# Kaixhin/Rainbow

Measured on AMD Instinct MI355X. Metric: gradient-steps/sec (batch=32, atoms=51), higher is better.
Workload: dtype f32; 1 GPU; pong-canonical-b32; architecture=canonical, batch_per_gpu=32, global_batch=32, atoms=51, actions=6, multi_step=3, replay_capacity_per_gpu=1000000, parallelism=single device

## Files before the change

### rainbow_amd/csrc/adam_body.h

```cpp
#pragma once
#include "rb_common.h"

struct ClipAdamArgs {
  float* p; float* g; float* m; float* v;
  int64_t n;
  const float* part; int nparts;
  float max_norm; float* norm_out;
  float w1, b2, w2, neg_step_size, bc2_sqrt, eps;
  const long long* step_dev;
  double lr, beta1, beta2;
  int64_t skip_lo4, skip_len4;
  const int32_t* batch_status;
  int64_t pair_mu4, pair_len4;
  unsigned hole_lo4, hole4;
  int pair_blk0;
  int pair_f4, pair_split_row;
  const float* pair_eout;
  const float* pair_ein;
  int32_t* pair_clipped;
};
__device__ __forceinline__ void rb_adam_elem(float& p, float& g, float& m, float& v, float coef, const ClipAdamArgs& a) {
  g = g * coef;
  m = fmaf(a.w1, g - m, m);
  v = v * a.b2 + a.w2 * g * g;
  const float denom = sqrtf(v) / a.bc2_sqrt + a.eps;
  p = p + a.neg_step_size * (m / denom);
}
__device__ __forceinline__ void rb_adam_quad(float4& P, float4& G, float4& M, float4& V, float coef, const ClipAdamArgs& a) {
  rb_adam_elem(P.x, G.x, M.x, V.x, coef, a);
  rb_adam_elem(P.y, G.y, M.y, V.y, coef, a);
  rb_adam_elem(P.z, G.z, M.z, V.z, coef, a);
  rb_adam_elem(P.w, G.w, M.w, V.w, coef, a);
}

struct rb_adam_req {
  float status;
  unsigned st_lo, st_hi;
  float pv[16];
};
__device__ __forceinline__ void rb_adam_hosted_request(const ClipAdamArgs& a, rb_adam_req& q) {
  const unsigned T = blockDim.x;
  q.status = 0.0f;
  if (a.batch_status) q.status = rb_ld1_buf(rb_make_buf(a.batch_status), 0, 0);
  const rb_buf bs = rb_make_buf(a.step_dev);
  q.st_lo = __builtin_bit_cast(unsigned, rb_ld1_buf(bs, 0, 0)); q.st_hi = __builtin_bit_cast(unsigned, rb_ld1_buf(bs, 4, 0));
  const rb_buf bpart = rb_make_buf(a.part);
#pragma unroll
  for (int u = 0; u < 16; ++u) {
    const int i = (int)threadIdx.x + u * (int)T;
    q.pv[u] = rb_ld1_buf(bpart, 4u * (unsigned)(i < a.nparts ? i : a.nparts - 1), 0);
  }
}
__device__ __forceinline__ bool rb_adam_hosted_prologue(ClipAdamArgs& a, int eb, const rb_adam_req& q, float* s_red16, float* coef_out) {
  const unsigned T = blockDim.x;
  float acc = 0.0f;
#pragma unroll
  for (int u = 0; u < 16; ++u)
    if ((int)threadIdx.x + u * (int)T < a.nparts) acc += q.pv[u];
  {
    const rb_buf bpart = rb_make_buf(a.part);
    for (int i0 = (int)threadIdx.x + 16 * (int)T; i0 < a.nparts; i0 += 16 * (int)T) {
      float pv[16];
#pragma unroll
      for (int u = 0; u < 16; ++u) {
        const int i = i0 + u * (int)T;
        pv[u] = rb_ld1_buf(bpart, 4u * (unsigned)(i < a.nparts ? i : a.nparts - 1), 0);
      }
#pragma unroll
      for (int u = 0; u < 16; ++u)
        if (i0 + u * (int)T < a.nparts) acc += pv[u];
    }
  }
  if (threadIdx.x == 0) {
    const double t = (double)(long long)(((unsigned long long)q.st_hi << 32) | q.st_lo);
    const double bc1 = 1.0 - pow(a.beta1, t), bc2 = 1.0 - pow(a.beta2, t);
    s_red16[16] = (float)(-(a.lr / bc1));
    s_red16[17] = (float)sqrt(bc2);
  }
  acc = rb_block_sum(acc, s_red16);
  if (rb_wave_uniform(__builtin_bit_cast(int, q.status)) != 0) {
    if (eb == 0 && threadIdx.x == 0 && a.norm_out) rb_st1_wt(a.norm_out, 0, 0.0f);
    return false;
  }
  const float total = sqrtf(acc);
  float coef = a.max_norm / (total + 1e-6f);
  if (coef > 1.0f) coef = 1.0f;
  if (eb == 0 && threadIdx.x == 0 && a.norm_out) rb_st1_wt(a.norm_out, 0, total);
  a.neg_step_size = s_red16[16];
  a.bc2_sqrt = s_red16[17];
  *coef_out = coef;
  return true;
}

__device__ __forceinline__ void rb_adam_hosted_pairs(ClipAdamArgs& a, int eb, int pb, float* s_red16) {
  constexpr int PU = 2;
  const unsigned T = blockDim.x;
  const unsigned len4 = (unsigned)a.pair_len4, mu4 = (unsigned)a.pair_mu4;
  const unsigned base = (unsigned)pb * (T * PU) + threadIdx.x;
  rb_adam_req q;
  rb_adam_hosted_request(a, q);
  const rb_buf beo = rb_make_buf(a.pair_eout), bei = rb_make_buf(a.pair_ein);
  float4 E[PU];
  float eo[PU];
#pragma unroll
  for (int u = 0; u < PU; ++u) {
    unsigned j = base + u * T;
    if (j >= len4) j = len4 - 1;
    const unsigned row = j / (unsigned)a.pair_f4, cq = j - row * (unsigned)a.pair_f4;
    eo[u] = rb_ld1_buf(beo, 4 * row, 0);
    E[u] = rb_ld4_buf(bei, 16 * (cq + ((int)row >= a.pair_split_row ? (unsigned)a.pair_f4 : 0u)), 0);
  }
  const rb_buf bp = rb_make_buf(a.p), bg = rb_make_buf(a.g), bm = rb_make_buf(a.m), bv = rb_make_buf(a.v);
  float4 P[PU], G[PU], M[PU], V[PU], P2[PU], M2[PU], V2[PU];
#pragma unroll
  for (int u = 0; u < PU; ++u) {
    unsigned j = base + u * T;
    if (j >= len4) j = len4 - 1;
    const unsigned i = mu4 + j, i2 = i + len4;
    P[u] = rb_ld4_buf(bp, 16 * i, 0); G[u] = rb_ld4_buf(bg, 16 * i, 0);
    M[u] = rb_ld4_buf(bm, 16 * i, 0); V[u] = rb_ld4_buf(bv, 16 * i, 0);
    P2[u] = rb_ld4_buf(bp, 16 * i2, 0); M2[u] = rb_ld4_buf(bm, 16 * i2, 0); V2[u] = rb_ld4_buf(bv, 16 * i2, 0);
  }
  float coef;
  if (!rb_adam_hosted_prologue(a, eb, q, s_red16, &coef)) return;
  if (pb == 0 && threadIdx.x == 0 && a.pair_clipped) rb_st1_wt(reinterpret_cast<float*>(a.pair_clipped), 0, __builtin_bit_cast(float, coef < 1.0f ? 1 : 0));
#pragma unroll
  for (int u = 0; u < PU; ++u) {
    const unsigned j = base + u * T;
    if (j >= len4) continue;
    const unsigned i = mu4 + j, i2 = i + len4;
    float4 pr;
    pr.x = eo[u] * E[u].x; pr.y = eo[u] * E[u].y; pr.z = eo[u] * E[u].z; pr.w = eo[u] * E[u].w;
    float4 G2;
    G2.x = G[u].x * pr.x; G2.y = G[u].y * pr.y; G2.z = G[u].z * pr.z; G2.w = G[u].w * pr.w;
    rb_adam_quad(P[u], G[u], M[u], V[u], coef, a);
    rb_adam_quad(P2[u], G2, M2[u], V2[u], coef, a);
    rb_st4_wt(a.p, 16 * i, P[u]); rb_st4_wt(a.m, 16 * i, M[u]); rb_st4_wt(a.v, 16 * i, V[u]);
    rb_st4_wt(a.p, 16 * i2, P2[u]); rb_st4_wt(a.m, 16 * i2, M2[u]); rb_st4_wt(a.v, 16 * i2, V2[u]);
    if (coef < 1.0f) { rb_st4_wt(a.g, 16 * i, G[u]); rb_st4_wt(a.g, 16 * i2, G2); }
  }
}

template <int UNROLL>
__device__ __forceinline__ void rb_adam_hosted_block(const ClipAdamArgs* ad, int eb, int nblk, float* s_red16 ) {
  ClipAdamArgs a = rb_ld_uniform(ad);
  const int nplain = a.hole4 > 0 ? a.pair_blk0 : nblk;
  if (eb >= nplain) {
    rb_adam_hosted_pairs(a, eb, eb - nplain, s_red16);
    return;
  }
  const unsigned T = blockDim.x;
  const unsigned n4 = (unsigned)(a.n >> 2);
  const unsigned hole_lo = a.hole4 > 0 ? a.hole_lo4 : n4, hole = a.hole4;
  const unsigned nv4 = n4 - hole;
  auto real_of = [&](unsigned j) { return j < hole_lo ? j : j + hole; };
  const unsigned base = (unsigned)eb * (T * UNROLL) + threadIdx.x;
  const rb_buf bp = rb_make_buf(a.p), bg = rb_make_buf(a.g), bm = rb_make_buf(a.m), bv = rb_make_buf(a.v);
  rb_adam_req q;
  rb_adam_hosted_request(a, q);
  float4 P[UNROLL], G[UNROLL], M[UNROLL], V[UNROLL];
#pragma unroll
  for (int u = 0; u < UNROLL; ++u) {
    unsigned j = base + u * T;
    if (j >= nv4) j = nv4 > 0 ? nv4 - 1 : 0;
    const unsigned i = real_of(j);
    P[u] = rb_ld4_buf(bp, 16 * i, 0); G[u] = rb_ld4_buf(bg, 16 * i, 0);
    M[u] = rb_ld4_buf(bm, 16 * i, 0); V[u] = rb_ld4_buf(bv, 16 * i, 0);
  }
  float coef;
  if (!rb_adam_hosted_prologue(a, eb, q, s_red16, &coef)) return;
#pragma unroll
  for (int u = 0; u < UNROLL; ++u) {
    const unsigned j = base + u * T;
    if (j >= nv4) continue;
    const unsigned i = real_of(j);
    rb_adam_quad(P[u], G[u], M[u], V[u], coef, a);
    rb_st4_wt(a.p, 16 * i, P[u]); rb_st4_wt(a.m, 16 * i, M[u]); rb_st4_wt(a.v, 16 * i, V[u]);
    if (coef < 1.0f) rb_st4_wt(a.g, 16 * i, G[u]);
  }
  if (eb == nplain - 1) {
    const int64_t t = ((a.n >> 2) << 2) + threadIdx.x;
    if (t < a.n) {
      const unsigned o = (unsigned)(4 * t);
      float p = rb_ld1_buf(bp, o, 0), g = rb_ld1_buf(bg, o, 0), m = rb_ld1_buf(bm, o, 0), v = rb_ld1_buf(bv, o, 0);
      rb_adam_elem(p, g, m, v, coef, a);
      rb_st1_wt(a.p, o, p); rb_st1_wt(a.m, o, m); rb_st1_wt(a.v, o, v);
      if (coef < 1.0f) rb_st1_wt(a.g, o, g);
    }
  }
}

int rb_launch_adam_pending(const ClipAdamArgs* args_dev, int blocks, void* stream);
```

### rainbow_amd/csrc/learner_internal.h

```cpp
#pragma once
#include "conv_fwd.h"
#include "conv_dx.h"
#include "conv_dw.h"
#include "noise_body.h"
#include "adam_body.h"
#include "learner_problems.h"
#include "noisy_linear.h"
#include "fc_gemm.h"
#include "act_path.h"
#include "rb_common.h"

#include <stdlib.h>

#include <math.h>
#include <string.h>

#include <new>

#define RB_HEAD_MAX_NZ 1408
typedef ConvGeom<8, 4, 84, 20> GeomC1;
typedef ConvGeom<4, 2, 20, 9> GeomC2;
typedef ConvGeom<3, 1, 9, 7> GeomC3;
typedef ConvGeom<5, 5, 84, 16> GeomD1;
typedef ConvGeom<5, 5, 16, 3> GeomD2;
// ... 2 lines not shown

struct ConvLayer {
  int cin, cout, ks, s, ih, oh;
  int K() const { return cin * ks * ks; }
  int P() const { return oh * oh; }
  int IP() const { return ih * ih; }
};

struct Layout {
  int B, Z, A, H, F, NZ, hist, nconv;
  ConvLayer conv[3];
  int64_t conv_w[3], conv_b[3];
  int64_t h_mu, h_sigma, h_bmu, h_bsigma, z_mu, z_sigma, z_bmu, z_bsigma;
  int64_t n_params;
  int64_t h_ein, h_eout, z_ein, z_eout, n_noise;
};

static int64_t align64(int64_t x) { return (x + 63) / 64 * 64; }

static int make_layout(const rb_learner_config_t* c, Layout* L) {
  RB_REQUIRE(c != nullptr, "learner config is NULL");
  RB_REQUIRE(c->batch >= 1 && c->batch <= 1024, "batch must be in [1,1024]");
  RB_REQUIRE(c->atoms >= 2 && c->atoms <= 256, "atoms must be in [2,256]");
  RB_REQUIRE(c->actions >= 1 && c->actions <= 64, "actions must be in [1,64]");
  RB_REQUIRE(c->atoms * (c->actions + 1) <= RB_HEAD_MAX_NZ, "atoms*(actions+1) must be <= %d (head kernel LDS rows)", RB_HEAD_MAX_NZ);
  RB_REQUIRE(c->history >= 1 && c->history <= 16, "history must be in [1,16]");
  RB_REQUIRE(c->hidden >= 1 && c->hidden <= 8192, "hidden must be in [1,8192]");
  RB_REQUIRE(c->architecture == 0 || c->architecture == 1, "architecture must be 0 (canonical) or 1 (data-efficient)");
  RB_REQUIRE(c->multi_step >= 1, "multi_step must be >= 1");
  RB_REQUIRE(c->v_max > c->v_min, "v_max must exceed v_min");
  memset(L, 0, sizeof(*L));
  L->B = c->batch; L->Z = c->atoms; L->A = c->actions; L->H = c->hidden; L->hist = c->history;
  L->NZ = L->Z + L->A * L->Z;
  if (c->architecture == 0) {
    L->nconv = 3;
    L->conv[0] = ConvLayer{c->history, 32, 8, 4, 84, 20};
    L->conv[1] = ConvLayer{32, 64, 4, 2, 20, 9};
    L->conv[2] = ConvLayer{64, 64, 3, 1, 9, 7};
    L->F = 3136;
  } else {
    L->nconv = 2;
    L->conv[0] = ConvLayer{c->history, 32, 5, 5, 84, 16};
    L->conv[1] = ConvLayer{32, 64, 5, 5, 16, 3};
    L->F = 576;
  }
  int64_t off = 0;
  for (int l = 0; l < L->nconv; ++l) {
    L->conv_w[l] = off; off = align64(off + (int64_t)L->conv[l].cout * L->conv[l].K());
    L->conv_b[l] = off; off = align64(off + L->conv[l].cout);
  }
  const int64_t H2 = 2 * L->H;
  L->h_mu = off; off = align64(off + H2 * L->F);
  L->h_sigma = off; off = align64(off + H2 * L->F);
  L->h_bmu = off; off = align64(off + H2);
  L->h_bsigma = off; off = align64(off + H2);
  L->z_mu = off; off = align64(off + (int64_t)L->NZ * L->H);
  L->z_sigma = off; off = align64(off + (int64_t)L->NZ * L->H);
  L->z_bmu = off; off = align64(off + L->NZ);
  L->z_bsigma = off; off = align64(off + L->NZ);
  L->n_params = off;
  int64_t n = 0;
  L->h_ein = n; n = align64(n + 2 * (int64_t)L->F);
  L->h_eout = n; n = align64(n + H2);
  L->z_ein = n; n = align64(n + H2);
  L->z_eout = n; n = align64(n + L->NZ);
  L->n_noise = n;
  return RB_OK;
}


static NetPtrs net_ptrs(const Layout& L, const float* params, const float* noise) {
  NetPtrs p;
  for (int l = 0; l < 3; ++l) {
    p.conv_w[l] = l < L.nconv ? params + L.conv_w[l] : nullptr;
    p.conv_b[l] = l < L.nconv ? params + L.conv_b[l] : nullptr;
  }
  p.h_mu = params + L.h_mu; p.h_sigma = params + L.h_sigma; p.h_bmu = params + L.h_bmu; p.h_bsigma = params + L.h_bsigma;
  p.z_mu = params + L.z_mu; p.z_sigma = params + L.z_sigma; p.z_bmu = params + L.z_bmu; p.z_bsigma = params + L.z_bsigma;
  p.h_ein = noise + L.h_ein; p.h_eout = noise + L.h_eout; p.z_ein = noise + L.z_ein; p.z_eout = noise + L.z_eout;
  return p;
}

struct RbOpts {
  int generic, fc_gemm, implicit_small, xs, act_fused, spec_draw, spec_stall, img_fast, conv_multi, conv_full, t16, dx_ipb, dw_ipb0, dw_ipb1, dw_ipb2;
};
static const struct { const char* key; int RbOpts::*field; int dflt; const char* what; } rb_opt_table[] = {
  {"generic", &RbOpts::generic, 0, "1: every contraction on the gemm_core.h fallback; 2: the noisy-linear layers only"},
  {"fc_gemm", &RbOpts::fc_gemm, -1, "hidden layer on the LDS-tiled GEMMs of fc_gemm.h: -1 = by shape (from 128 rows per net on), 1 = always, 0 = never"},
  {"implicit_small", &RbOpts::implicit_small, 0, "test hook: RB_LEARNER_IMPLICIT_SIGMA on hidden layers of any size"},
  {"xs", &RbOpts::xs, 0, "row splits of the hidden layer's input gradient: 0 = derived from the hidden size (ceil(2H / 256), at most 4)"},
  {"act_fused", &RbOpts::act_fused, 1, "Agent.act as ONE launch (0: the per-layer launches)"},
  {"spec_draw", &RbOpts::spec_draw, 0, "the early draw (opt-in: only append-free loops ever arm it)"},
  {"spec_stall", &RbOpts::spec_stall, 0, "test hook: the early draw's go flag is never stored, the gate in front of the pair expires"},
  {"img_fast", &RbOpts::img_fast, 1, "image-fastest block order of the conv launches (0: the order that image counts off a multiple of 8 get)"},
  {"conv_multi", &RbOpts::conv_multi, -1, "images per workgroup of the conv forward: -1 = by shape (from 256 images on), 0 = one"},
  {"conv_full", &RbOpts::conv_full, 1, "the first layer's whole-image kernel at large batches (0: the chunked kernel)"},
  {"t16", &RbOpts::t16, 1, "the canonical first layer's u8 forward on whole-K 16x16x4 tiles (0: the split-K kernel that history < 4 gets)"},
  {"dx_ipb", &RbOpts::dx_ipb, 0, "images per workgroup of the conv input gradients: 0 = by shape (from batch 64 on)"},
  {"dw_ipb0", &RbOpts::dw_ipb0, 0, "images per workgroup of conv layer 0 in the weight-gradient launch: 0 = by shape"},
  {"dw_ipb1", &RbOpts::dw_ipb1, 0, "... of conv layer 1"},
  {"dw_ipb2", &RbOpts::dw_ipb2, 0, "... of conv layer 2"},
};
static int rb_opts_parse(const char* s, RbOpts* o) {
  for (const auto& row : rb_opt_table) o->*row.field = row.dflt;
  while (s && *s) {
    const char* e = strchr(s, ',');
    const size_t n = e ? (size_t)(e - s) : strlen(s);
    const char* eq = (const char*)memchr(s, '=', n);
    RB_REQUIRE(eq != nullptr && eq > s, "RB_OPTS: entry '%.*s' is not key=value", (int)n, s);
    const size_t kl = (size_t)(eq - s);
    int RbOpts::*field = nullptr;
    for (const auto& row : rb_opt_table)
      if (strlen(row.key) == kl && strncmp(row.key, s, kl) == 0) field = row.field;
    RB_REQUIRE(field != nullptr, "RB_OPTS: unknown key '%.*s'", (int)kl, s);
    char* end = nullptr;
    const long v = strtol(eq + 1, &end, 10);
    RB_REQUIRE(end == s + n && end > eq + 1, "RB_OPTS: key '%.*s' needs an integer value", (int)kl, s);
    o->*field = (int)v;
    s = e ? e + 1 : s + n;
  }
  return RB_OK;
}

struct LearnerCaps {
  int fast_fc;
  int fast_conv;
  int hs, xs, ws[3];
  int wT[3];
  int gemm_ws;
};

struct rb_learner {
  rb_learner_config_t cfg;
  Layout L;
  float *p_online, *p_target, *grads, *n_online, *n_target;
  uint64_t seed;
  uint64_t noise_epoch;
  float* act[3];
  float* dact[3];
  float* hpart;
  float* h;
  float *feat_b, *h_b;
  float *feat_s, *h_s;
  int rows_s_cap;
  float* logits;
  float* dlogits;
  float* dlogitsT;
  float* dh;
  float* dhT;
  float* dfeat_part;
  int lazy_dfeat;
  int lazy_splits;
  RbOpts opt;
  float* gemm_part;
  unsigned* gemm_ctr;
  float* dw_part[3];
  float* conv_wT[3];
  float* log_ps_a;
  float* pns_a;
  float* m;
  int32_t* a_star;
  float* support;
  float* zero_noise;
  float* norm_part;
  int norm_conv_base;
  int norm_slots;
  unsigned long long* noise_ctr;
  NoiseJob* job_dev;
  unsigned* act_ctr;
  unsigned act_epoch;
  int n_cu;
  int rows_cap;
  LearnerCaps caps;
  int dw_slices[3];
  ImgSrc cur_src;
  int sink_done;
  const int32_t* batch_status;
  rb_replay_t* sink;
  const int64_t* sink_idx;
  int world;
  float* fact_local;
  const float* fact_all;
  int64_t fact_off[6];
  int64_t fact_stride;
// ... 36 lines not shown
```

### rainbow_amd/csrc/optimizer_host.h

```cpp
#pragma once
#include "learner_plan.h"

static int materialize_sigma(rb_learner* l, hipStream_t stream) {
  if (!l->sigma_implicit) return RB_OK;
  const Layout& L = l->L;
  const NetPtrs sn = net_ptrs(L, l->p_online, l->noise_snap);
  const int64_t len4 = (int64_t)2 * L.H * L.F / 4;
  RB_LAUNCH(k_materialize_sigma, dim3((unsigned)rb_div_up(len4, 256 * 4)), dim3(256), stream, l->grads, L.h_mu / 4, len4, L.F / 4, L.H,
            sn.h_eout, sn.h_ein, (const int32_t*)(l->status_copy + 2));
  RB_LAUNCH_CHECK();
  l->sigma_implicit = 0;
  return RB_OK;
}

static int flush_update(rb_learner* l, hipStream_t stream) {
  if (!l->adam_pending) return RB_OK;
  FusedDwAdamArgs f;
  memset(&f, 0, sizeof(f));
  ClipAdamArgs a = l->adam_args_host;
  int blocks = l->adam_blocks;
  if (a.pair_len4 > 0) {
    const int rc = rb_launch_adam_pending(l->adam_args_dev, blocks, stream);
    if (rc != RB_OK) return rc;
    l->adam_pending = 0;
    return RB_OK;
  }
  RB_LAUNCH_T("clip_adam:k_clip_adam", (k_clip_adam<4, true, false>), dim3((unsigned)blocks), dim3(256), stream, a, f);
  RB_LAUNCH_CHECK();
  l->adam_pending = 0;
  return RB_OK;
}

static int sumsq_pass(rb_learner* l, hipStream_t stream, int* nparts) {
  const int64_t n = l->L.n_params;
  *nparts = plan_sumsq_blocks(n);
  RB_LAUNCH(k_sumsq, dim3((unsigned)*nparts), dim3(256), stream, (const float*)l->grads, n, l->norm_part);
  RB_LAUNCH_CHECK();
  return RB_OK;
}

static bool attach_pending_pass(rb_learner* l, const rb_noise_job_t* job_in, int32_t batch, rb_noise_job_t* job_out) {
  memcpy(job_out, job_in, sizeof(*job_out));
  if (!l->adam_pending || batch > 256) return false;
  NoiseJob* nj = reinterpret_cast<NoiseJob*>(job_out);
  nj->adam_dev = l->adam_args_dev; nj->adam_blocks = l->adam_blocks;
  return true;
}

static int clip_adam_impl(rb_learner* l, float max_norm, float* exp_avg, float* exp_avg_sq, double lr, double beta1, double beta2,
                          double eps, int64_t step, float* norm_dev, hipStream_t stream, bool defer) {
  RB_REQUIRE(exp_avg != nullptr && exp_avg_sq != nullptr, "rb_learner_clip_adam: NULL moment buffer");
  RB_REQUIRE(step >= 1 || (step == 0 && l->step_ctr), "rb_learner_clip_adam: step is 1-based (0 = take it from the device counter set "
             "with rb_learner_set_step_counter)");
  const int64_t n = l->L.n_params;
  int nparts = l->norm_slots;
  if (!(max_norm < INFINITY) && norm_dev == nullptr) {
    nparts = 0;
  } else if (nparts <= 0) {
    const int rcs = sumsq_pass(l, stream, &nparts);
    if (rcs != RB_OK) return rcs;
  }
  l->norm_slots = 0;
  ClipAdamArgs a;
  memset(&a, 0, sizeof(a));
  a.p = l->p_online; a.g = l->grads; a.m = exp_avg; a.v = exp_avg_sq; a.n = n;
  a.part = l->norm_part; a.nparts = nparts; a.max_norm = max_norm; a.norm_out = norm_dev;
  const double bc1 = 1.0 - pow(beta1, (double)step), bc2 = 1.0 - pow(beta2, (double)step);
  a.w1 = (float)(1.0 - beta1); a.b2 = (float)beta2; a.w2 = (float)(1.0 - beta2);
  a.neg_step_size = (float)(-(lr / bc1)); a.bc2_sqrt = (float)sqrt(bc2); a.eps = (float)eps;
  a.step_dev = step == 0 ? l->step_ctr : nullptr; a.lr = lr; a.beta1 = beta1; a.beta2 = beta2;
  a.batch_status = l->status_copy;
  const int64_t n4 = n >> 2;
  RB_REQUIRE(n * 4 < (int64_t)0x7fffffff, "rb_learner_clip_adam: the flat parameter buffer must be smaller than 2 GiB");
  FusedDwAdamArgs f;
  memset(&f, 0, sizeof(f));
  a.skip_lo4 = 0; a.skip_len4 = 0;
  if (l->dw_deferred) {
    const Layout& L = l->L;
    const NetPtrs on = net_ptrs(L, l->p_online, l->n_online);
    FcDwPlan hp = fc_dw_plan(l, on, 1, l->dh, l->act[L.nconv - 1], L.B, 0);
    f.dw = hp.a;
    f.mu_off = L.h_mu; f.sigma_off = L.h_sigma;
    f.dw_x = hp.dw_x; f.n_tile_blocks = 2 * hp.dw_x * hp.dw_y;
    f.write_grads = (l->flags & RB_LEARNER_WRITE_FUSED_GRADS) ? 1 : 0;
    a.skip_lo4 = L.h_mu >> 2; a.skip_len4 = (L.h_bmu - L.h_mu) >> 2;
    const unsigned grid = (unsigned)(f.n_tile_blocks + rb_div_up(n4 - a.skip_len4 > 0 ? n4 - a.skip_len4 : 1, 256 * 4));
    RB_LAUNCH_T("clip_adam:k_clip_adam", (k_clip_adam<4, true, true>), dim3(grid), dim3(256), stream, a, f);
    l->dw_deferred = 0;
  } else {
    unsigned grid = (unsigned)rb_div_up(n4 > 0 ? n4 : 1, 256 * 4);
    const bool will_defer = defer && a.step_dev != nullptr && a.nparts > 0 && l->adam_args_dev != nullptr;
    if (l->sigma_implicit && will_defer) {
      const Layout& L = l->L;
      const NetPtrs sn = net_ptrs(L, l->p_online, l->noise_snap);
      a.pair_mu4 = L.h_mu / 4; a.pair_len4 = (int64_t)2 * L.H * L.F / 4;
      a.pair_f4 = L.F / 4; a.pair_split_row = L.H; a.pair_eout = sn.h_eout; a.pair_ein = sn.h_ein;
      a.pair_clipped = l->status_copy + 2;
      a.hole_lo4 = (unsigned)a.pair_mu4; a.hole4 = (unsigned)(2 * a.pair_len4);
      a.pair_blk0 = (int)rb_div_up(n4 - 2 * a.pair_len4 > 0 ? n4 - 2 * a.pair_len4 : 1, 256 * 4);
      grid = (unsigned)(a.pair_blk0 + rb_div_up(a.pair_len4, 256 * 2));
    } else if (l->sigma_implicit) {
      const int rcm = materialize_sigma(l, stream);
      if (rcm != RB_OK) return rcm;
    }
    if (will_defer) {
      if (!l->adam_args_valid || memcmp(&a, &l->adam_args_host, sizeof(a)) != 0) {
        RB_LAUNCH(k_store_adam_args, dim3(1), dim3(64), stream, a, l->adam_args_dev);
        RB_LAUNCH_CHECK();
        memcpy(&l->adam_args_host, &a, sizeof(a));
        l->adam_args_valid = 1;
      }
      l->adam_pending = 1;
      l->adam_blocks = (int)grid;
      return RB_OK;
    }
    RB_LAUNCH_T("clip_adam:k_clip_adam", (k_clip_adam<4, true, false>), dim3(grid), dim3(256), stream, a, f);
  }
  RB_LAUNCH_CHECK();
  return RB_OK;
}

extern "C" {

int rb_learner_flush(rb_learner_t* l, rb_stream_t stream) {
  RB_REQUIRE(l != nullptr, "rb_learner_flush: NULL handle");
  const int rc = flush_update(l, (hipStream_t)stream);
  if (rc != RB_OK) return rc;
  return materialize_sigma(l, (hipStream_t)stream);
}

int rb_learner_attach_pending(rb_learner_t* l, const rb_noise_job_t* job_in, int32_t batch, rb_noise_job_t* job_out) {
  if (!l || !job_in || !job_out) { rb_set_error("rb_learner_attach_pending: NULL argument"); return RB_ERR_INVALID; }
  return attach_pending_pass(l, job_in, batch, job_out) ? 1 : 0;
}
int rb_learner_pending_launched(rb_learner_t* l) {
  RB_REQUIRE(l != nullptr, "rb_learner_pending_launched: NULL handle");
  l->adam_pending = 0;
  return RB_OK;
}
int rb_debug_adam_pass(int32_t form, float* p, float* g, float* m, float* v, int64_t n, const float* part, int32_t nparts,
                       float max_norm, float* norm_out, const long long* step_dev, int64_t step, double lr, double beta1,
                       double beta2, double eps, const int32_t* batch_status, int64_t pair_mu4, int64_t pair_len4, int32_t pair_f4,
                       int32_t pair_split_row, const float* pair_eout, const float* pair_ein, int32_t* pair_clipped, void* args_dev,
                       rb_stream_t stream_) {
  hipStream_t stream = (hipStream_t)stream_;
  RB_REQUIRE(p && g && m && v && part && n >= 0 && n * 4 < (int64_t)0x7fffffff && nparts > 0, "rb_debug_adam_pass: bad buffers");
  RB_REQUIRE(form == 0 ? (step >= 1 && pair_len4 == 0) : (form == 1 && step_dev && args_dev), "rb_debug_adam_pass: bad form");
  static_assert(sizeof(ClipAdamArgs) <= 256, "rb_debug_adam_pass: args_dev is documented as 256 bytes");
  ClipAdamArgs a;
  memset(&a, 0, sizeof(a));
  a.p = p; a.g = g; a.m = m; a.v = v; a.n = n;
  a.part = part; a.nparts = nparts; a.max_norm = max_norm; a.norm_out = norm_out;
  const double bc1 = 1.0 - pow(beta1, (double)step), bc2 = 1.0 - pow(beta2, (double)step);
  a.w1 = (float)(1.0 - beta1); a.b2 = (float)beta2; a.w2 = (float)(1.0 - beta2);
  a.neg_step_size = (float)(-(lr / bc1)); a.bc2_sqrt = (float)sqrt(bc2); a.eps = (float)eps;
  a.step_dev = form == 1 ? step_dev : nullptr; a.lr = lr; a.beta1 = beta1; a.beta2 = beta2;
  a.batch_status = batch_status;
  const int64_t n4 = n >> 2;
  unsigned grid = (unsigned)rb_div_up(n4 > 0 ? n4 : 1, 256 * 4);
  if (form == 0) {
    FusedDwAdamArgs f;
    memset(&f, 0, sizeof(f));
    RB_LAUNCH((k_clip_adam<4, true, false>), dim3(grid), dim3(256), stream, a, f);
    RB_LAUNCH_CHECK();
    return RB_OK;
  }
  if (pair_len4 > 0) {
    RB_REQUIRE(pair_mu4 >= 0 && pair_mu4 + 2 * pair_len4 <= n4 && pair_f4 > 0 && pair_len4 % pair_f4 == 0 && pair_eout && pair_ein,
               "rb_debug_adam_pass: bad pair range");
    a.pair_mu4 = pair_mu4; a.pair_len4 = pair_len4; a.pair_f4 = pair_f4; a.pair_split_row = pair_split_row;
    a.pair_eout = pair_eout; a.pair_ein = pair_ein; a.pair_clipped = pair_clipped;
    a.hole_lo4 = (unsigned)pair_mu4; a.hole4 = (unsigned)(2 * pair_len4);
    a.pair_blk0 = (int)rb_div_up(n4 - 2 * pair_len4 > 0 ? n4 - 2 * pair_len4 : 1, 256 * 4);
    grid = (unsigned)(a.pair_blk0 + rb_div_up(pair_len4, 256 * 2));
  }
  RB_LAUNCH(k_store_adam_args, dim3(1), dim3(64), stream, a, reinterpret_cast<ClipAdamArgs*>(args_dev));
  RB_LAUNCH_CHECK();
  return rb_launch_adam_pending(reinterpret_cast<const ClipAdamArgs*>(args_dev), (int)grid, stream);
}

int rb_learner_clip_adam_deferred(rb_learner_t* l, float max_norm, float* exp_avg, float* exp_avg_sq, double lr, double beta1,
                                  double beta2, double eps, int64_t step, float* norm_dev, rb_stream_t stream) {
  RB_REQUIRE(l != nullptr, "rb_learner_clip_adam_deferred: NULL handle");
  const int rc = flush_update(l, (hipStream_t)stream);
  if (rc != RB_OK) return rc;
  return clip_adam_impl(l, max_norm, exp_avg, exp_avg_sq, lr, beta1, beta2, eps, step, norm_dev, (hipStream_t)stream,
                        (l->flags & RB_LEARNER_DEFER_UPDATE) != 0);
}

int rb_learner_clip_grad(rb_learner_t* l, float max_norm, float* norm_dev, rb_stream_t stream) {
  RB_REQUIRE(l != nullptr, "rb_learner_clip_grad: NULL handle");
  RB_FLUSH_UPDATE(l, stream);
  RB_MATERIALIZE_SIGMA(l, stream);
  if (l->dw_deferred) {
    rb_set_error("rb_learner_clip_grad: the last learn call left the hidden layer's weight gradient to the fused optimiser "
                 "pass (RB_LEARNER_FUSE_FC_H_DW); call rb_learner_clip_adam, or clear the flag before learning");
    return RB_ERR_STATE;
  }
  const int64_t n = l->L.n_params;
  int nblocks = plan_sumsq_blocks(n);
  int nparts = l->norm_slots;
  if (nparts > 0) {
    if (nblocks > 256) nblocks = 256;
  } else {
    const int rcs = sumsq_pass(l, (hipStream_t)stream, &nparts);
    if (rcs != RB_OK) return rcs;
  }
  l->norm_slots = 0;
  RB_LAUNCH(k_clip_scale, dim3((unsigned)nblocks), dim3(256), stream, l->grads, n, (const float*)l->norm_part, nparts,
            max_norm, norm_dev);
  RB_LAUNCH_CHECK();
  return RB_OK;
}

int rb_learner_clip_adam(rb_learner_t* l, float max_norm, float* exp_avg, float* exp_avg_sq, double lr, double beta1,
                         double beta2, double eps, int64_t step, float* norm_dev, rb_stream_t stream) {
  RB_REQUIRE(l != nullptr, "rb_learner_clip_adam: NULL handle");
  const int rc = flush_update(l, (hipStream_t)stream);
  if (rc != RB_OK) return rc;
  return clip_adam_impl(l, max_norm, exp_avg, exp_avg_sq, lr, beta1, beta2, eps, step, norm_dev, (hipStream_t)stream, false);
}

}
```

### rainbow_amd/csrc/replay.hip

```cpp
#include "noise_body.h"
#include "adam_body.h"
#include "replay_internal.h"
#include "replay_search.h"
#include "replay_append.h"
#include "replay_spec.h"
#include "replay_sample.h"
#include "replay_view.h"

#include <stdlib.h>
#include <string.h>

#include <new>

struct rb_replay {
  int64_t capacity;
  int32_t history, n;
  int32_t levels;
  int32_t streams;
  int64_t tree_start;
  int64_t tree_len;
  double omega;
  uint64_t seed;
  float scaling[64];
  float* tree;
// ... 352 lines not shown
int rb_replay_append_streams_dev(rb_replay_t* r, const float* states_dev, int32_t* timesteps_dev, const int32_t* actions_dev,
                                 const float* rewards_dev, const uint8_t* nonterminals_dev, rb_stream_t stream) {
  AppendRoundDev a;
  a.timestep = timesteps_dev; a.action = actions_dev; a.reward = rewards_dev; a.nonterminal = nonterminals_dev;
  const bool have = timesteps_dev && actions_dev && rewards_dev && nonterminals_dev;
  return append_round(r, "rb_replay_append_streams_dev", "append:k_append_streams_dev", states_dev, have ? &a : nullptr, stream);
}

int rb_replay_set_beta_source(rb_replay_t* r, const float* neg_beta_dev) {
  RB_REQUIRE(r != nullptr, "rb_replay_set_beta_source: NULL handle");
  r->neg_beta_dev = neg_beta_dev;
  return RB_OK;
}

int rb_replay_find(rb_replay_t* r, const double* values_dev, int32_t n, float* probs_dev, int64_t* data_idx_dev,
                   int64_t* tree_idx_dev, rb_stream_t stream) {
  RB_REQUIRE(r && values_dev && probs_dev && data_idx_dev && tree_idx_dev, "rb_replay_find: NULL argument");
  RB_SPEC_JOIN(r);
  if (n <= 0) return RB_OK;
  RB_LAUNCH(k_find, dim3((unsigned)rb_div_up(n, 256)), dim3(256), stream, view_of(r), values_dev, n, probs_dev,
            data_idx_dev, tree_idx_dev);
  RB_LAUNCH_CHECK();
  return RB_OK;
}

static int launch_gather(const ReplayView& v, int32_t batch, const int32_t* win, uint8_t* states_dev, uint8_t* next_states_dev,
                         rb_stream_t stream) {
  if (!states_dev || !next_states_dev) return RB_OK;
  RB_LAUNCH(k_gather_stacks, dim3((unsigned)(batch * 2 * v.history)), dim3(256), stream, v, batch, win, states_dev, next_states_dev);
  RB_LAUNCH_CHECK();
  return RB_OK;
}

static int sample_impl(rb_replay_t* r, int32_t batch, double priority_weight, const double* unit_uniforms_dev,
                       int32_t max_attempts, int64_t* tree_idx_dev, uint8_t* states_dev, uint8_t* next_states_dev,
                       int64_t* actions_dev, float* returns_dev, float* nonterminals_dev, float* weights_dev,
                       const rb_noise_job_t* noise_job, rb_stream_t stream) {
  RB_REQUIRE(r && tree_idx_dev && actions_dev && returns_dev && nonterminals_dev && weights_dev,
             "rb_replay_sample: NULL argument");
  RB_REQUIRE(batch >= 1 && batch <= r->max_batch, "rb_replay_sample: batch must be in [1,%d]", r->max_batch);
  RB_REQUIRE(max_attempts >= 1, "rb_replay_sample: max_attempts must be >= 1");
  RB_REQUIRE(r->capacity > (int64_t)r->history + r->n,
             "rb_replay_sample: capacity must exceed history + multi_step (no window can clear the write head otherwise: "
             "the reference's rejection loop, memory.py:128-132, would never end)");
  const int accept_armed = r->spec_accept_armed;
  r->spec_accept_armed = 0;
  int spec_mode = 0;
  int win_set = 0;
  if (r->spec_inflight) {
    const bool same = accept_armed && !rb_stream_capturing(stream) && unit_uniforms_dev == nullptr && r->spec_args.batch == batch && r->spec_args.beta == priority_weight &&
                      r->spec_args.max_attempts == max_attempts && r->spec_args.tree_idx == tree_idx_dev &&
                      r->spec_args.actions == actions_dev && r->spec_args.returns == returns_dev &&
                      r->spec_args.nonterm == nonterminals_dev && r->spec_args.weights == weights_dev;
    spec_mode = same ? 2 : 3;
    if (same) win_set = r->spec_args.win_set;
    r->spec_inflight = 0;
  }
  r->win_sel = win_set;
  ++r->mutations;
  int32_t* const win_cur = win_of(r, win_set);
  const ReplayView v = view_of(r);
  const float neg_beta = (float)(-priority_weight);
  NoiseJob job;
  memset(&job, 0, sizeof(job));
  unsigned blocks = 1;
  if (noise_job) {
    memcpy(&job, noise_job, sizeof(job));
    RB_REQUIRE(job.noise && job.ctr && job.nblk > 0 && job.nets >= 1 && job.dev, "rb_replay_sample_fused_noise: empty noise job");
    blocks += (unsigned)(job.nblk * job.nets);
  }
  const int noise_blocks = (int)blocks - 1;
  int threads = (int)(rb_div_up(batch, 64) * 64);
  if (threads < 256) threads = 256;
  const int window = r->history + r->n;
  const ClipAdamArgs* adam_dev = nullptr;
  if (noise_job && job.adam_dev && job.adam_blocks > 0) {
    RB_REQUIRE(threads == 256, "rb_replay_sample_fused_noise: the hosted optimiser pass needs a 256-thread sampler launch (batch <= 256)");
    adam_dev = static_cast<const ClipAdamArgs*>(job.adam_dev);
  }
  const bool hosted = adam_dev && window <= 24;
  const bool wide = threads > 256 || hosted;
  RB_REQUIRE(!wide || window <= 24, "rb_replay_sample: the 1024-thread sampler (batch > 256) supports history + multi_step <= 24");
  if (hosted) {
    blocks += (unsigned)((job.adam_blocks * 4 + RB_HOST_AU_WIDE - 1) / RB_HOST_AU_WIDE);
  } else if (adam_dev) {
    const int rc = rb_launch_adam_pending(adam_dev, job.adam_blocks, stream);
    if (rc != RB_OK) return rc;
    adam_dev = nullptr;
  }
  const int lds_top = 1;
  auto launch = [&](auto kernel) {
    RB_LAUNCH_T("sample:k_sample", kernel, dim3(blocks), dim3(threads), stream, v, batch, neg_beta, r->neg_beta_dev, unit_uniforms_dev,
                max_attempts, r->seed, r->scaling_dev, tree_idx_dev, win_cur, actions_dev, returns_dev, nonterminals_dev, weights_dev,
                job.dev, job.noise, job.noise2, job.ctr, r->fail_host, lds_top, noise_blocks, adam_dev, r->spec_res, r->spec_epoch,
                spec_mode);
  };
  if (wide) launch(k_sample<1024, RB_HOST_AU_WIDE>);
  else launch(k_sample<256, 8>);
  RB_LAUNCH_CHECK();
  return launch_gather(v, batch, win_cur, states_dev, next_states_dev, stream);
}

int rb_replay_sample(rb_replay_t* r, int32_t batch, double priority_weight, const double* unit_uniforms_dev,
                     int32_t max_attempts, int64_t* tree_idx_dev, uint8_t* states_dev, uint8_t* next_states_dev,
                     int64_t* actions_dev, float* returns_dev, float* nonterminals_dev, float* weights_dev,
                     rb_stream_t stream) {
  return sample_impl(r, batch, priority_weight, unit_uniforms_dev, max_attempts, tree_idx_dev, states_dev, next_states_dev,
                     actions_dev, returns_dev, nonterminals_dev, weights_dev, nullptr, stream);
}

int rb_replay_sample_fused_noise(rb_replay_t* r, int32_t batch, double priority_weight, const double* unit_uniforms_dev,
                                 int32_t max_attempts, int64_t* tree_idx_dev, uint8_t* states_dev, uint8_t* next_states_dev,
                                 int64_t* actions_dev, float* returns_dev, float* nonterminals_dev, float* weights_dev,
                                 const rb_noise_job_t* noise_job, rb_stream_t stream) {
  RB_REQUIRE(noise_job != nullptr, "rb_replay_sample_fused_noise: noise_job is NULL");
  return sample_impl(r, batch, priority_weight, unit_uniforms_dev, max_attempts, tree_idx_dev, states_dev, next_states_dev,
                     actions_dev, returns_dev, nonterminals_dev, weights_dev, noise_job, stream);
}

static int rb_update_impl(rb_replay_t* r, const int64_t* tree_idx_dev, const float* values_dev, int32_t n,
                          int32_t apply_pow, rb_stream_t stream) {
  RB_REQUIRE(r && tree_idx_dev && values_dev, "rb_replay_update: NULL argument");
  RB_REQUIRE(n >= 1 && n <= 1024, "rb_replay_update: n must be in [1,1024]");
  RB_SPEC_JOIN(r);
  ++r->mutations;
  int threads = (int)(rb_div_up(n, 64) * 64);
  if (threads < 256) threads = 256;
  RB_LAUNCH(k_update, dim3(1), dim3(threads), stream, view_of(r), tree_idx_dev, values_dev, n, apply_pow, r->omega);
  RB_LAUNCH_CHECK();
  return RB_OK;
}

int rb_replay_update_leaves(rb_replay_t* r, const int64_t* tree_idx_dev, const float* values_dev, int32_t n,
                            rb_stream_t stream) {
  return rb_update_impl(r, tree_idx_dev, values_dev, n, 0, stream);
}

int rb_replay_update_priorities(rb_replay_t* r, const int64_t* tree_idx_dev, const float* losses_dev, int32_t n,
                                rb_stream_t stream) {
  return rb_update_impl(r, tree_idx_dev, losses_dev, n, 1, stream);
}

int rb_replay_update_sample(rb_replay_t* r, const int64_t* upd_tree_idx_dev, const float* upd_losses_dev, int32_t upd_n,
                            int32_t batch, double priority_weight, const double* unit_uniforms_dev, int32_t max_attempts,
                            int64_t* tree_idx_dev, uint8_t* states_dev, uint8_t* next_states_dev, int64_t* actions_dev,
                            float* returns_dev, float* nonterminals_dev, float* weights_dev, rb_stream_t stream) {
  RB_REQUIRE(r && upd_tree_idx_dev && upd_losses_dev, "rb_replay_update_sample: NULL argument");
  RB_REQUIRE(upd_n >= 1 && upd_n <= 1024, "rb_replay_update_sample: upd_n must be in [1,1024]");
  if (upd_n > 64 || batch > 256) {
    const int rc = rb_update_impl(r, upd_tree_idx_dev, upd_losses_dev, upd_n, 1, stream);
    if (rc != RB_OK) return rc;
    return sample_impl(r, batch, priority_weight, unit_uniforms_dev, max_attempts, tree_idx_dev, states_dev, next_states_dev,
                       actions_dev, returns_dev, nonterminals_dev, weights_dev, nullptr, stream);
  }
  RB_REQUIRE(tree_idx_dev && actions_dev && returns_dev && nonterminals_dev && weights_dev, "rb_replay_update_sample: NULL argument");
  RB_REQUIRE(batch >= 1, "rb_replay_update_sample: batch must be in [1,%d]", r->max_batch);
  RB_REQUIRE(max_attempts >= 1, "rb_replay_update_sample: max_attempts must be >= 1");
  RB_REQUIRE(r->capacity > (int64_t)r->history + r->n, "rb_replay_update_sample: capacity must exceed history + multi_step");
  RB_SPEC_JOIN(r);
  ++r->mutations;
  r->win_sel = 0;
  const ReplayView v = view_of(r);
  const float neg_beta = (float)(-priority_weight);
  RB_LAUNCH_T("sample:k_update_sample", k_update_sample, dim3(1), dim3(256), stream, v, upd_tree_idx_dev, upd_losses_dev, upd_n, 1, r->omega,
              batch, neg_beta, r->neg_beta_dev, unit_uniforms_dev, max_attempts, r->seed, r->scaling_dev, tree_idx_dev, r->win, actions_dev,
              returns_dev, nonterminals_dev, weights_dev, r->fail_host, (SpecResult*)nullptr, 0u);
  RB_LAUNCH_CHECK();
// ... 59 lines not shown
```

Baseline: 6559 gradient-steps/s.

## Cap hosted Adam pass grid at resident slots and loop virtual blocks per workgroup

Converts the hosted optimiser pass to a grid-stride form: the number of workgroups is capped at the resident slots (4 per CU minus reserved sampler/noise blocks), and each workgroup loops over several virtual Adam blocks. The gradient-norm reduction prologue then runs once per workgroup instead of once per virtual block. This avoids redundant partial-sum reductions and launch tail from many short blocks. The cost is less memory-level parallelism per workgroup and serialised load/update iterations. It also changes how the sampler's fused launch sizes its hosted Adam block count.

```diff
diff --git a/rainbow_amd/csrc/adam_body.h b/rainbow_amd/csrc/adam_body.h
--- a/rainbow_amd/csrc/adam_body.h
+++ b/rainbow_amd/csrc/adam_body.h
@@ -14,6 +14,7 @@
   int64_t pair_mu4, pair_len4;
   unsigned hole_lo4, hole4;
   int pair_blk0;
+  int nvirt;
   int pair_f4, pair_split_row;
   const float* pair_eout;
   const float* pair_ein;
@@ -92,37 +93,43 @@
   return true;
 }
 
-__device__ __forceinline__ void rb_adam_hosted_pairs(ClipAdamArgs& a, int eb, int pb, float* s_red16) {
-  constexpr int PU = 2;
+struct rb_adam_bufs { rb_buf p, g, m, v; };
+
+#define RB_ADAM_PU 2
+struct rb_adam_pair_regs {
+  float4 E[RB_ADAM_PU];
+  float eo[RB_ADAM_PU];
+  float4 P[RB_ADAM_PU], G[RB_ADAM_PU], M[RB_ADAM_PU], V[RB_ADAM_PU], P2[RB_ADAM_PU], M2[RB_ADAM_PU], V2[RB_ADAM_PU];
+};
+__device__ __forceinline__ void rb_adam_pair_load(const ClipAdamArgs& a, const rb_adam_bufs& b, int pb, rb_adam_pair_regs& r) {
+  constexpr int PU = RB_ADAM_PU;
   const unsigned T = blockDim.x;
   const unsigned len4 = (unsigned)a.pair_len4, mu4 = (unsigned)a.pair_mu4;
   const unsigned base = (unsigned)pb * (T * PU) + threadIdx.x;
-  rb_adam_req q;
-  rb_adam_hosted_request(a, q);
   const rb_buf beo = rb_make_buf(a.pair_eout), bei = rb_make_buf(a.pair_ein);
-  float4 E[PU];
-  float eo[PU];
 #pragma unroll
   for (int u = 0; u < PU; ++u) {
     unsigned j = base + u * T;
     if (j >= len4) j = len4 - 1;
     const unsigned row = j / (unsigned)a.pair_f4, cq = j - row * (unsigned)a.pair_f4;
-    eo[u] = rb_ld1_buf(beo, 4 * row, 0);
-    E[u] = rb_ld4_buf(bei, 16 * (cq + ((int)row >= a.pair_split_row ? (unsigned)a.pair_f4 : 0u)), 0);
-  }
-  const rb_buf bp = rb_make_buf(a.p), bg = rb_make_buf(a.g), bm = rb_make_buf(a.m), bv = rb_make_buf(a.v);
-  float4 P[PU], G[PU], M[PU], V[PU], P2[PU], M2[PU], V2[PU];
+    r.eo[u] = rb_ld1_buf(beo, 4 * row, 0);
+    r.E[u] = rb_ld4_buf(bei, 16 * (cq + ((int)row >= a.pair_split_row ? (unsigned)a.pair_f4 : 0u)), 0);
+  }
 #pragma unroll
   for (int u = 0; u < PU; ++u) {
     unsigned j = base + u * T;
     if (j >= len4) j = len4 - 1;
     const unsigned i = mu4 + j, i2 = i + len4;
-    P[u] = rb_ld4_buf(bp, 16 * i, 0); G[u] = rb_ld4_buf(bg, 16 * i, 0);
-    M[u] = rb_ld4_buf(bm, 16 * i, 0); V[u] = rb_ld4_buf(bv, 16 * i, 0);
-    P2[u] = rb_ld4_buf(bp, 16 * i2, 0); M2[u] = rb_ld4_buf(bm, 16 * i2, 0); V2[u] = rb_ld4_buf(bv, 16 * i2, 0);
-  }
-  float coef;
-  if (!rb_adam_hosted_prologue(a, eb, q, s_red16, &coef)) return;
+    r.P[u] = rb_ld4_buf(b.p, 16 * i, 0); r.G[u] = rb_ld4_buf(b.g, 16 * i, 0);
+    r.M[u] = rb_ld4_buf(b.m, 16 * i, 0); r.V[u] = rb_ld4_buf(b.v, 16 * i, 0);
+    r.P2[u] = rb_ld4_buf(b.p, 16 * i2, 0); r.M2[u] = rb_ld4_buf(b.m, 16 * i2, 0); r.V2[u] = rb_ld4_buf(b.v, 16 * i2, 0);
+  }
+}
+__device__ __forceinline__ void rb_adam_pair_update(const ClipAdamArgs& a, int pb, float coef, rb_adam_pair_regs& r) {
+  constexpr int PU = RB_ADAM_PU;
+  const unsigned T = blockDim.x;
+  const unsigned len4 = (unsigned)a.pair_len4, mu4 = (unsigned)a.pair_mu4;
+  const unsigned base = (unsigned)pb * (T * PU) + threadIdx.x;
   if (pb == 0 && threadIdx.x == 0 && a.pair_clipped) rb_st1_wt(reinterpret_cast<float*>(a.pair_clipped), 0, __builtin_bit_cast(float, coef < 1.0f ? 1 : 0));
 #pragma unroll
   for (int u = 0; u < PU; ++u) {
@@ -130,59 +137,57 @@
     if (j >= len4) continue;
     const unsigned i = mu4 + j, i2 = i + len4;
     float4 pr;
-    pr.x = eo[u] * E[u].x; pr.y = eo[u] * E[u].y; pr.z = eo[u] * E[u].z; pr.w = eo[u] * E[u].w;
+    pr.x = r.eo[u] * r.E[u].x; pr.y = r.eo[u] * r.E[u].y; pr.z = r.eo[u] * r.E[u].z; pr.w = r.eo[u] * r.E[u].w;
     float4 G2;
-    G2.x = G[u].x * pr.x; G2.y = G[u].y * pr.y; G2.z = G[u].z * pr.z; G2.w = G[u].w * pr.w;
-    rb_adam_quad(P[u], G[u], M[u], V[u], coef, a);
-    rb_adam_quad(P2[u], G2, M2[u], V2[u], coef, a);
-    rb_st4_wt(a.p, 16 * i, P[u]); rb_st4_wt(a.m, 16 * i, M[u]); rb_st4_wt(a.v, 16 * i, V[u]);
-    rb_st4_wt(a.p, 16 * i2, P2[u]); rb_st4_wt(a.m, 16 * i2, M2[u]); rb_st4_wt(a.v, 16 * i2, V2[u]);
-    if (coef < 1.0f) { rb_st4_wt(a.g, 16 * i, G[u]); rb_st4_wt(a.g, 16 * i2, G2); }
-  }
-}
-
-template <int UNROLL>
-__device__ __forceinline__ void rb_adam_hosted_block(const ClipAdamArgs* ad, int eb, int nblk, float* s_red16 ) {
-  ClipAdamArgs a = rb_ld_uniform(ad);
-  const int nplain = a.hole4 > 0 ? a.pair_blk0 : nblk;
-  if (eb >= nplain) {
-    rb_adam_hosted_pairs(a, eb, eb - nplain, s_red16);
-    return;
-  }
+    G2.x = r.G[u].x * pr.x; G2.y = r.G[u].y * pr.y; G2.z = r.G[u].z * pr.z; G2.w = r.G[u].w * pr.w;
+    rb_adam_quad(r.P[u], r.G[u], r.M[u], r.V[u], coef, a);
+    rb_adam_quad(r.P2[u], G2, r.M2[u], r.V2[u], coef, a);
+    rb_st4_wt(a.p, 16 * i, r.P[u]); rb_st4_wt(a.m, 16 * i, r.M[u]); rb_st4_wt(a.v, 16 * i, r.V[u]);
+    rb_st4_wt(a.p, 16 * i2, r.P2[u]); rb_st4_wt(a.m, 16 * i2, r.M2[u]); rb_st4_wt(a.v, 16 * i2, r.V2[u]);
+    if (coef < 1.0f) { rb_st4_wt(a.g, 16 * i, r.G[u]); rb_st4_wt(a.g, 16 * i2, G2); }
+  }
+}
+
+template <int UNROLL>
+struct rb_adam_plain_regs { float4 P[UNROLL], G[UNROLL], M[UNROLL], V[UNROLL]; };
+template <int UNROLL>
+__device__ __forceinline__ void rb_adam_plain_load(const ClipAdamArgs& a, const rb_adam_bufs& b, int eb, rb_adam_plain_regs<UNROLL>& r) {
   const unsigned T = blockDim.x;
   const unsigned n4 = (unsigned)(a.n >> 2);
   const unsigned hole_lo = a.hole4 > 0 ? a.hole_lo4 : n4, hole = a.hole4;
   const unsigned nv4 = n4 - hole;
-  auto real_of = [&](unsigned j) { return j < hole_lo ? j : j + hole; };
   const unsigned base = (unsigned)eb * (T * UNROLL) + threadIdx.x;
-  const rb_buf bp = rb_make_buf(a.p), bg = rb_make_buf(a.g), bm = rb_make_buf(a.m), bv = rb_make_buf(a.v);
-  rb_adam_req q;
-  rb_adam_hosted_request(a, q);
-  float4 P[UNROLL], G[UNROLL], M[UNROLL], V[UNROLL];
 #pragma unroll
   for (int u = 0; u < UNROLL; ++u) {
     unsigned j = base + u * T;
     if (j >= nv4) j = nv4 > 0 ? nv4 - 1 : 0;
-    const unsigned i = real_of(j);
-    P[u] = rb_ld4_buf(bp, 16 * i, 0); G[u] = rb_ld4_buf(bg, 16 * i, 0);
-    M[u] = rb_ld4_buf(bm, 16 * i, 0); V[u] = rb_ld4_buf(bv, 16 * i, 0);
-  }
-  float coef;
-  if (!rb_adam_hosted_prologue(a, eb, q, s_red16, &coef)) return;
+    const unsigned i = j < hole_lo ? j : j + hole;
+    r.P[u] = rb_ld4_buf(b.p, 16 * i, 0); r.G[u] = rb_ld4_buf(b.g, 16 * i, 0);
+    r.M[u] = rb_ld4_buf(b.m, 16 * i, 0); r.V[u] = rb_ld4_buf(b.v, 16 * i, 0);
+  }
+}
+template <int UNROLL>
+__device__ __forceinline__ void rb_adam_plain_update(const ClipAdamArgs& a, const rb_adam_bufs& b, int eb, int nplain, float coef,
+                                                     rb_adam_plain_regs<UNROLL>& r) {
+  const unsigned T = blockDim.x;
+  const unsigned n4 = (unsigned)(a.n >> 2);
+  const unsigned hole_lo = a.hole4 > 0 ? a.hole_lo4 : n4, hole = a.hole4;
+  const unsigned nv4 = n4 - hole;
+  const unsigned base = (unsigned)eb * (T * UNROLL) + threadIdx.x;
 #pragma unroll
   for (int u = 0; u < UNROLL; ++u) {
     const unsigned j = base + u * T;
     if (j >= nv4) continue;
-    const unsigned i = real_of(j);
-    rb_adam_quad(P[u], G[u], M[u], V[u], coef, a);
-    rb_st4_wt(a.p, 16 * i, P[u]); rb_st4_wt(a.m, 16 * i, M[u]); rb_st4_wt(a.v, 16 * i, V[u]);
-    if (coef < 1.0f) rb_st4_wt(a.g, 16 * i, G[u]);
+    const unsigned i = j < hole_lo ? j : j + hole;
+    rb_adam_quad(r.P[u], r.G[u], r.M[u], r.V[u], coef, a);
+    rb_st4_wt(a.p, 16 * i, r.P[u]); rb_st4_wt(a.m, 16 * i, r.M[u]); rb_st4_wt(a.v, 16 * i, r.V[u]);
+    if (coef < 1.0f) rb_st4_wt(a.g, 16 * i, r.G[u]);
   }
   if (eb == nplain - 1) {
     const int64_t t = ((a.n >> 2) << 2) + threadIdx.x;
     if (t < a.n) {
       const unsigned o = (unsigned)(4 * t);
-      float p = rb_ld1_buf(bp, o, 0), g = rb_ld1_buf(bg, o, 0), m = rb_ld1_buf(bm, o, 0), v = rb_ld1_buf(bv, o, 0);
+      float p = rb_ld1_buf(b.p, o, 0), g = rb_ld1_buf(b.g, o, 0), m = rb_ld1_buf(b.m, o, 0), v = rb_ld1_buf(b.v, o, 0);
       rb_adam_elem(p, g, m, v, coef, a);
       rb_st1_wt(a.p, o, p); rb_st1_wt(a.m, o, m); rb_st1_wt(a.v, o, v);
       if (coef < 1.0f) rb_st1_wt(a.g, o, g);
@@ -190,4 +195,47 @@
   }
 }
 
+template <int UNROLL>
+__device__ __forceinline__ void rb_adam_hosted_block(const ClipAdamArgs* ad, int w, int G, float* s_red16 ) {
+  ClipAdamArgs a = rb_ld_uniform(ad);
+  const int nvirt = a.nvirt;
+  const int nplain = a.hole4 > 0 ? a.pair_blk0 : nvirt;
+  rb_adam_bufs b;
+  b.p = rb_make_buf(a.p); b.g = rb_make_buf(a.g); b.m = rb_make_buf(a.m); b.v = rb_make_buf(a.v);
+  float coef;
+  int eb = w;
+  if (eb >= nplain) {
+    rb_adam_req q;
+    rb_adam_hosted_request(a, q);
+    rb_adam_pair_regs r;
+    rb_adam_pair_load(a, b, eb - nplain, r);
+    if (!rb_adam_hosted_prologue(a, eb, q, s_red16, &coef)) return;
+    rb_adam_pair_update(a, eb - nplain, coef, r);
+    for (eb += G; eb < nvirt; eb += G) {
+      rb_adam_pair_load(a, b, eb - nplain, r);
+      rb_adam_pair_update(a, eb - nplain, coef, r);
+    }
+    return;
+  }
+  {
+    rb_adam_req q;
+    rb_adam_hosted_request(a, q);
+    rb_adam_plain_regs<UNROLL> r;
+    rb_adam_plain_load<UNROLL>(a, b, eb, r);
+    if (!rb_adam_hosted_prologue(a, eb, q, s_red16, &coef)) return;
+    rb_adam_plain_update<UNROLL>(a, b, eb, nplain, coef, r);
+    for (eb += G; eb < nplain; eb += G) {
+      rb_adam_plain_load<UNROLL>(a, b, eb, r);
+      rb_adam_plain_update<UNROLL>(a, b, eb, nplain, coef, r);
+    }
+  }
+  if (eb < nvirt) {
+    rb_adam_pair_regs r;
+    for (; eb < nvirt; eb += G) {
+      rb_adam_pair_load(a, b, eb - nplain, r);
+      rb_adam_pair_update(a, eb - nplain, coef, r);
+    }
+  }
+}
+
 int rb_launch_adam_pending(const ClipAdamArgs* args_dev, int blocks, void* stream);
diff --git a/rainbow_amd/csrc/learner_internal.h b/rainbow_amd/csrc/learner_internal.h
--- a/rainbow_amd/csrc/learner_internal.h
+++ b/rainbow_amd/csrc/learner_internal.h
@@ -108,7 +108,7 @@
 }
 
 struct RbOpts {
-  int generic, fc_gemm, implicit_small, xs, act_fused, spec_draw, spec_stall, img_fast, conv_multi, conv_full, t16, dx_ipb, dw_ipb0, dw_ipb1, dw_ipb2;
+  int generic, fc_gemm, implicit_small, xs, act_fused, spec_draw, spec_stall, img_fast, conv_multi, conv_full, t16, dx_ipb, dw_ipb0, dw_ipb1, dw_ipb2, adam_slots;
 };
 static const struct { const char* key; int RbOpts::*field; int dflt; const char* what; } rb_opt_table[] = {
   {"generic", &RbOpts::generic, 0, "1: every contraction on the gemm_core.h fallback; 2: the noisy-linear layers only"},
@@ -126,6 +126,7 @@
   {"dw_ipb0", &RbOpts::dw_ipb0, 0, "images per workgroup of conv layer 0 in the weight-gradient launch: 0 = by shape"},
   {"dw_ipb1", &RbOpts::dw_ipb1, 0, "... of conv layer 1"},
   {"dw_ipb2", &RbOpts::dw_ipb2, 0, "... of conv layer 2"},
+  {"adam_slots", &RbOpts::adam_slots, 0, "workgroups of the hosted optimiser pass: 0 = 4 per CU (its resident slots); test hook: fewer give small buffers several shares per workgroup"},
 };
 static int rb_opts_parse(const char* s, RbOpts* o) {
   for (const auto& row : rb_opt_table) o->*row.field = row.dflt;
diff --git a/rainbow_amd/csrc/optimizer_host.h b/rainbow_amd/csrc/optimizer_host.h
--- a/rainbow_amd/csrc/optimizer_host.h
+++ b/rainbow_amd/csrc/optimizer_host.h
@@ -10,6 +10,22 @@
             sn.h_eout, sn.h_ein, (const int32_t*)(l->status_copy + 2));
   RB_LAUNCH_CHECK();
   l->sigma_implicit = 0;
+  return RB_OK;
+}
+
+static int plan_adam_grid(int nvirt, int n_cu, int adam_slots, int reserved) {
+  int slots = adam_slots > 0 ? adam_slots : 4 * n_cu - reserved;
+  if (slots < 1) slots = 1;
+  return nvirt < slots ? nvirt : slots;
+}
+static int device_cu_count(int* cus) {
+#if defined(RB_HOST_INTERP)
+  *cus = 8;
+#else
+  int dev = 0;
+  RB_HIP_TRY(hipGetDevice(&dev));
+  RB_HIP_TRY(hipDeviceGetAttribute(cus, hipDeviceAttributeMultiprocessorCount, dev));
+#endif
   return RB_OK;
 }
 
@@ -25,7 +41,7 @@
     l->adam_pending = 0;
     return RB_OK;
   }
-  RB_LAUNCH_T("clip_adam:k_clip_adam", (k_clip_adam<4, true, false>), dim3((unsigned)blocks), dim3(256), stream, a, f);
+  RB_LAUNCH_T("clip_adam:k_clip_adam", (k_clip_adam<4, true, false>), dim3((unsigned)a.nvirt), dim3(256), stream, a, f);
   RB_LAUNCH_CHECK();
   l->adam_pending = 0;
   return RB_OK;
@@ -43,7 +59,8 @@
   memcpy(job_out, job_in, sizeof(*job_out));
   if (!l->adam_pending || batch > 256) return false;
   NoiseJob* nj = reinterpret_cast<NoiseJob*>(job_out);
-  nj->adam_dev = l->adam_args_dev; nj->adam_blocks = l->adam_blocks;
+  nj->adam_dev = l->adam_args_dev;
+  nj->adam_blocks = plan_adam_grid(l->adam_args_host.nvirt, l->n_cu, l->opt.adam_slots, 1 + nj->nblk * nj->nets);
   return true;
 }
 
@@ -103,6 +120,7 @@
       const int rcm = materialize_sigma(l, stream);
       if (rcm != RB_OK) return rcm;
     }
+    a.nvirt = (int)grid;
     if (will_defer) {
       if (!l->adam_args_valid || memcmp(&a, &l->adam_args_host, sizeof(a)) != 0) {
         RB_LAUNCH(k_store_adam_args, dim3(1), dim3(64), stream, a, l->adam_args_dev);
@@ -111,7 +129,7 @@
         l->adam_args_valid = 1;
       }
       l->adam_pending = 1;
-      l->adam_blocks = (int)grid;
+      l->adam_blocks = plan_adam_grid((int)grid, l->n_cu, l->opt.adam_slots, 0);
       return RB_OK;
     }
     RB_LAUNCH_T("clip_adam:k_clip_adam", (k_clip_adam<4, true, false>), dim3(grid), dim3(256), stream, a, f);
@@ -174,9 +192,16 @@
     a.pair_blk0 = (int)rb_div_up(n4 - 2 * pair_len4 > 0 ? n4 - 2 * pair_len4 : 1, 256 * 4);
     grid = (unsigned)(a.pair_blk0 + rb_div_up(pair_len4, 256 * 2));
   }
+  a.nvirt = (int)grid;
+  RbOpts opt;
+  int rc = rb_opts_parse(getenv("RB_OPTS"), &opt);
+  if (rc != RB_OK) return rc;
+  int cus = 0;
+  rc = device_cu_count(&cus);
+  if (rc != RB_OK) return rc;
   RB_LAUNCH(k_store_adam_args, dim3(1), dim3(64), stream, a, reinterpret_cast<ClipAdamArgs*>(args_dev));
   RB_LAUNCH_CHECK();
-  return rb_launch_adam_pending(reinterpret_cast<const ClipAdamArgs*>(args_dev), (int)grid, stream);
+  return rb_launch_adam_pending(reinterpret_cast<const ClipAdamArgs*>(args_dev), plan_adam_grid((int)grid, cus, opt.adam_slots, 0), stream);
 }
 
 int rb_learner_clip_adam_deferred(rb_learner_t* l, float max_norm, float* exp_avg, float* exp_avg_sq, double lr, double beta1,
diff --git a/rainbow_amd/csrc/replay.hip b/rainbow_amd/csrc/replay.hip
--- a/rainbow_amd/csrc/replay.hip
+++ b/rainbow_amd/csrc/replay.hip
@@ -458,7 +458,7 @@
   const bool wide = threads > 256 || hosted;
   RB_REQUIRE(!wide || window <= 24, "rb_replay_sample: the 1024-thread sampler (batch > 256) supports history + multi_step <= 24");
   if (hosted) {
-    blocks += (unsigned)((job.adam_blocks * 4 + RB_HOST_AU_WIDE - 1) / RB_HOST_AU_WIDE);
+    blocks += (unsigned)job.adam_blocks;
   } else if (adam_dev) {
     const int rc = rb_launch_adam_pending(adam_dev, job.adam_blocks, stream);
     if (rc != RB_OK) return rc;
```

New measurement: 6434 gradient-steps/s. 0.981x the previous value.
